# daniloceano/LorenzCycleToolkit

Measured on NVIDIA B200. Metric: LEC timesteps/s (all terms), 0.25°×37-lvl ERA5 shape; % of HBM roofline, higher is better.
Workload: dtype f32

## Files before the change

### lorenzcycletoolkit_b200/csrc/lec_engine.cu

```cuda
#include <algorithm>
#include <cmath>
#include <cstdio>
#include <cstdlib>
#include <cstring>
#include <string>
#include <vector>

#include "../../include/lec_b200.h"
#include "lec_common.cuh"
#include "lec_finalize.cuh"
#include "lec_row_moments.cuh"
#include "lec_row_tile.cuh"
#include "lec_row_narrow.cuh"
#include "lec_diag850.cuh"
#include "lec_ingest.cuh"

using namespace lec;

#ifndef LEC_TILE_DEFAULT
#define LEC_TILE_DEFAULT 1
#endif
#ifndef LEC_TILE_ROWS_DEFAULT
#define LEC_TILE_ROWS_DEFAULT 15
#endif
// ... 25 lines not shown
  int force_narrow_g = 0;
  double* d_rec = nullptr;
  double* d_fin = nullptr;
  StepDev* d_steps = nullptr;
  StepDev* h_steps = nullptr;
  cudaEvent_t ev_steps[2] = {nullptr, nullptr};
  bool steps_pending[2] = {false, false};
  int batch_parity = 0;
  int max_steps = 0, max_ny = 0;
  size_t elem = 4;
  std::vector<double> lon_deg, lat_deg, rlon, rlat, coslat, plev;
  void* stage[2][5] = {{nullptr}};
  long long stage_slots = 0;
  void* raw_stage[2] = {nullptr, nullptr};
  size_t raw_stage_bytes = 0;
  cudaStream_t s_ingest = nullptr;
  cudaEvent_t ev_raw_ready[2] = {nullptr, nullptr}, ev_raw_free[2] = {nullptr, nullptr}, ev_ingested = nullptr;
  long long raw_seq = 0;
  int* d_maps = nullptr;
  double* d_out_terms = nullptr;
  double* d_out_levels = nullptr;
  int* d_out_flags = nullptr;
  long long out_cap = 0;
  double* bnd_user = nullptr;
  double* d_out_bnd = nullptr;
  long long bnd_cap = 0;
  cudaStream_t s_copy = nullptr, s_comp = nullptr;
  cudaEvent_t ev_copied[2] = {nullptr, nullptr}, ev_done[2] = {nullptr, nullptr};
  std::vector<cudaEvent_t> ev_pool;
  int ev_used = 0;
  cudaEvent_t ev_call0 = nullptr, ev_call1 = nullptr;
  bool call_timed = false;
  bool accumulate_timing = false;
  long long launches = 0;
  lec_dispatch dispatch{};
  bool dispatched = false;
  std::string err;
};

namespace {

#if LEC_TILE_DEFAULT
const char* kVersion = "lec_b200 0.2 (sm_100a; rows=tile)";
#else
const char* kVersion = "lec_b200 0.2 (sm_100a; rows=direct)";
#endif

#define CK(call)                                                                   \
  do {                                                                             \
    cudaError_t e__ = (call);                                                      \
    if (e__ != cudaSuccess) {                                                      \
      h->err = std::string(#call) + ": " + cudaGetErrorString(e__);                \
      return LEC_ERR_CUDA;                                                         \
    }                                                                              \
  } while (0)

inline void grad_interior(const double* x, int i, double& a, double& b, double& c) {
  const double hs = x[i] - x[i - 1], hd = x[i + 1] - x[i];
  if (hs == hd) {
    a = -1.0 / (2.0 * hs); b = 0.0; c = 1.0 / (2.0 * hs);
  } else {
    a = -hd / (hs * (hd + hs)); b = (hd - hs) / (hd * hs); c = hs / (hd * (hd + hs));
  }
}

int lon_mode(const lec_handle* h) {
  const bool m64 = h->desc.dtype == LEC_F64 || h->desc.math == LEC_MATH_F64;
  const int need = m64 ? 2 : 1;
  if (h->g.lon_uniform >= need) return 0;
  return h->g.stencil_uniform >= need ? 1 : 2;
}

template <typename FT, typename CT, int VEC, bool COMP>
void launch_rows_c(const RowParams& rp, int lonw, long long grid, cudaStream_t st) {
  if (lonw == 0) lec_row_moments_kernel<FT, CT, VEC, 0, COMP><<<(unsigned)grid, kRowThreads, 0, st>>>(rp);
  else if (lonw == 1) lec_row_moments_kernel<FT, CT, VEC, 1, COMP><<<(unsigned)grid, kRowThreads, 0, st>>>(rp);
  else lec_row_moments_kernel<FT, CT, VEC, 2, COMP><<<(unsigned)grid, kRowThreads, 0, st>>>(rp);
}
template <typename FT, typename CT, int VEC>
void launch_rows_t(const RowParams& rp, int lonw, bool comp, long long grid, cudaStream_t st) {
  if constexpr (sizeof(CT) == 4) {
    if (comp) { launch_rows_c<FT, CT, VEC, true>(rp, lonw, grid, st); return; }
  }
  launch_rows_c<FT, CT, VEC, false>(rp, lonw, grid, st);
}

void launch_rows(const lec_handle* h, const RowParams& rp, bool vec, bool comp, long long grid, cudaStream_t st) {
  const bool f64 = h->desc.dtype == LEC_F64;
  const bool m64 = f64 || h->desc.math == LEC_MATH_F64;
  const int lonw = lon_mode(h);
  if (f64) {
    if (vec) launch_rows_t<double, double, 2>(rp, lonw, comp, grid, st);
    else launch_rows_t<double, double, 1>(rp, lonw, comp, grid, st);
  } else if (m64) {
    if (vec) launch_rows_t<float, double, 4>(rp, lonw, comp, grid, st);
    else launch_rows_t<float, double, 1>(rp, lonw, comp, grid, st);
  } else {
    if (vec) launch_rows_t<float, float, 4>(rp, lonw, comp, grid, st);
    else launch_rows_t<float, float, 1>(rp, lonw, comp, grid, st);
  }
}

template <typename FT, typename CT, int VEC, bool COMP, typename ST>
void launch_narrow_c(const RowParams& rp, bool table, int G, long long grid, cudaStream_t st) {
#define LEC_NARROW(LW, GG) lec_row_moments_narrow_kernel<FT, CT, VEC, LW, GG, COMP, ST><<<(unsigned)grid, kNarrowThreads, 0, st>>>(rp)
  if (table) { if (G == 16) LEC_NARROW(2, 16); else if (G == 8) LEC_NARROW(2, 8); else LEC_NARROW(2, 4); }
  else { if (G == 16) LEC_NARROW(0, 16); else if (G == 8) LEC_NARROW(0, 8); else LEC_NARROW(0, 4); }
#undef LEC_NARROW
}
template <typename FT, typename CT, int VEC, typename ST = FT>
void launch_narrow_t(const RowParams& rp, bool table, bool comp, int G, long long grid, cudaStream_t st) {
  if constexpr (sizeof(CT) == 4) {
    if (comp) { launch_narrow_c<FT, CT, VEC, true, ST>(rp, table, G, grid, st); return; }
  }
  launch_narrow_c<FT, CT, VEC, false, ST>(rp, table, G, grid, st);
}

typedef CUresult (*EncodeTiledFn)(CUtensorMap*, CUtensorMapDataType, cuuint32_t, void*, const cuuint64_t*,
                                  const cuuint64_t*, const cuuint32_t*, const cuuint32_t*, CUtensorMapInterleave,
                                  CUtensorMapSwizzle, CUtensorMapL2promotion, CUtensorMapFloatOOBfill);

EncodeTiledFn encode_tiled_fn() {
  static EncodeTiledFn fn = nullptr;
  if (!fn) {
    void* ptr = nullptr;
    cudaDriverEntryPointQueryResult qres;
    if (cudaGetDriverEntryPoint("cuTensorMapEncodeTiled", &ptr, cudaEnableDefault, &qres) == cudaSuccess &&
        qres == cudaDriverEntryPointSuccess)
      fn = reinterpret_cast<EncodeTiledFn>(ptr);
  }
  return fn;
}

bool make_map(CUtensorMap* m, const void* base, int esize, int nlon, int nlat, int nlev, int nslots, int bx, int by,
              int promo = 3) {
  EncodeTiledFn enc = encode_tiled_fn();
  if (!enc) return false;
  const cuuint64_t e = (cuuint64_t)esize;
  const cuuint64_t dims[4] = {(cuuint64_t)nlon, (cuuint64_t)nlat, (cuuint64_t)nlev, (cuuint64_t)nslots};
  const cuuint64_t strides[3] = {nlon * e, (cuuint64_t)nlat * nlon * e, (cuuint64_t)nlev * nlat * nlon * e};
  const cuuint32_t box[4] = {(cuuint32_t)bx, (cuuint32_t)by, 1, 1};
  const cuuint32_t estr[4] = {1, 1, 1, 1};
  const CUtensorMapDataType dt = esize == 8 ? CU_TENSOR_MAP_DATA_TYPE_FLOAT64
                                 : esize == 4 ? CU_TENSOR_MAP_DATA_TYPE_FLOAT32 : CU_TENSOR_MAP_DATA_TYPE_UINT16;
  return enc(m, dt, 4, const_cast<void*>(base),
             dims, strides, box, estr, CU_TENSOR_MAP_INTERLEAVE_NONE, CU_TENSOR_MAP_SWIZZLE_NONE,
             promo == 0 ? CU_TENSOR_MAP_L2_PROMOTION_NONE : promo == 1 ? CU_TENSOR_MAP_L2_PROMOTION_L2_64B
             : promo == 2 ? CU_TENSOR_MAP_L2_PROMOTION_L2_128B : CU_TENSOR_MAP_L2_PROMOTION_L2_256B,
             CU_TENSOR_MAP_FLOAT_OOB_FILL_NONE) == CUDA_SUCCESS;
}

template <typename FT, typename CT, int R, int S, bool COMP, int GL = 32, int MINB = 1, typename ST = FT>
cudaError_t launch_tile_c(const TmaMaps& maps, const RowParams& rp, int lonw, int grid, cudaStream_t st) {
  using G = TileGeom<FT, R, S, GL, ST>;
  cudaError_t e = cudaSuccess;
#define LEC_TILE_LAUNCH(LW, TB, SMEM)                                                                             \
  do {                                                                                                            \
    e = cudaFuncSetAttribute(lec_row_moments_tile_kernel<FT, CT, LW, R, S, COMP, TB, GL, MINB, ST>,          \
                             cudaFuncAttributeMaxDynamicSharedMemorySize, SMEM);                                  \
    if (e == cudaSuccess) lec_row_moments_tile_kernel<FT, CT, LW, R, S, COMP, TB, GL, MINB, ST><<<grid, G::threads, SMEM, st>>>(maps, rp); \
  } while (0)
  if constexpr (GL != 32) {
    if (lonw == 0) LEC_TILE_LAUNCH(0, false, G::smem_bytes);
    else LEC_TILE_LAUNCH(2, false, G::smem_bytes);
  } else {
    const int tab_bytes = (sizeof(ST) == sizeof(FT) ? (rp.g.nlon + 3) & ~3 : rp.pk.ntab) * 4;
    if (lonw == 0) LEC_TILE_LAUNCH(0, false, G::smem_bytes);
    else if (lonw == 1) {
      if (sizeof(CT) == 4 && sizeof(FT) == 4 && G::smem_bytes + tab_bytes <= 227 * 1024) LEC_TILE_LAUNCH(1, true, G::smem_bytes + tab_bytes);
      else LEC_TILE_LAUNCH(1, false, G::smem_bytes);
    } else LEC_TILE_LAUNCH(2, false, G::smem_bytes);
  }
#undef LEC_TILE_LAUNCH
  return e != cudaSuccess ? e : cudaGetLastError();
}

template <typename FT, typename CT>
cudaError_t launch_tile_t(const TmaMaps& maps, const RowParams& rp, int lonw, bool comp, int rows, int grid,
                          cudaStream_t st) {
  if constexpr (sizeof(CT) == 4) {
    if (comp) return launch_tile_c<FT, CT, 11, 4, true>(maps, rp, lonw, grid, st);
#ifdef LEC_TILE_ALL_SHAPES
    if (rows == 8) return launch_tile_c<FT, CT, 8, 5, false>(maps, rp, lonw, grid, st);
    if (rows == 11) return launch_tile_c<FT, CT, 11, 4, false>(maps, rp, lonw, grid, st);
    if (rows == 12) return launch_tile_c<FT, CT, 12, 4, false>(maps, rp, lonw, grid, st);
#endif
    return launch_tile_c<FT, CT, 15, 3, false>(maps, rp, lonw, grid, st);
  } else if constexpr (sizeof(FT) == 4) {
    return launch_tile_c<FT, CT, 7, 6, false>(maps, rp, lonw, grid, st);
  } else {
    return launch_tile_c<FT, CT, 11, 4, false>(maps, rp, lonw, grid, st);
  }
}

template <typename FT, typename CT>
cudaError_t launch_tile_packed(const TmaMaps& maps, const RowParams& rp, int lonw, bool comp, int grid, cudaStream_t st) {
  if constexpr (sizeof(CT) == 4) {
    if (comp) return launch_tile_c<FT, CT, 11, 7, true, 32, 1, short>(maps, rp, lonw, grid, st);
    return launch_tile_c<FT, CT, 11, 7, false, 32, 1, short>(maps, rp, lonw, grid, st);
  } else if constexpr (sizeof(FT) == 4) {
    return launch_tile_c<FT, CT, 7, 8, false, 32, 1, short>(maps, rp, lonw, grid, st);
  } else {
    return launch_tile_c<FT, CT, 11, 8, false, 32, 1, short>(maps, rp, lonw, grid, st);
  }
}

cudaEvent_t next_event(lec_handle* h) {
  if (h->ev_used == (int)h->ev_pool.size()) {
    cudaEvent_t e;
    if (cudaEventCreate(&e) != cudaSuccess) return nullptr;
    h->ev_pool.push_back(e);
  }
  return h->ev_pool[h->ev_used++];
}

int build_step(const lec_handle* h, const lec_step& s, int nslots, StepDev& d) {
  const int nlon = h->desc.nlon, nlat = h->desc.nlat;
  if (s.slot < 0 || s.slot >= nslots || s.slot_m < 0 || s.slot_m >= nslots || s.slot_p < 0 ||
      s.slot_p >= nslots)
    return LEC_ERR_BOUNDS;
  if (s.i0 < 0 || s.i1 >= nlon || s.j0 < 0 || s.j1 >= nlat) return LEC_ERR_BOUNDS;
  if (s.i1 - s.i0 < 1 || s.j1 - s.j0 < 1) return LEC_ERR_DEGENERATE;
  if (s.j1 - s.j0 + 1 > h->max_ny) return LEC_ERR_BOUNDS;
  const double* x = h->lon_deg.data();
  const double* y = h->lat_deg.data();
  const double* rl = h->rlon.data();
  const double* rp = h->rlat.data();
  d.slot = s.slot; d.slot_m = s.slot_m; d.slot_p = s.slot_p;
  d.i0 = s.i0; d.i1 = s.i1; d.j0 = s.j0; d.j1 = s.j1; d.rec_base = 0;
  const double q0 = kCp * h->g.scale[0], qv = q0 * h->g.scale[2];
  d.ct_m = q0 * s.ct_m; d.ct_p = q0 * s.ct_p; d.ct_s = q0 * (s.ct_m + s.ct_0 + s.ct_p);
  const double unit = kDeg2Rad * kRe;
  d.cxW = 1.0 / ((x[s.i0 + 1] - x[s.i0]) * unit);
  d.cxE = 1.0 / ((x[s.i1] - x[s.i1 - 1]) * unit);
  d.cyS = qv / ((y[s.j0 + 1] - y[s.j0]) * unit);
  d.cyN = qv / ((y[s.j1] - y[s.j1 - 1]) * unit);
  d.wW = 0.5 * (rl[s.i0 + 1] - rl[s.i0]);
  d.wE = 0.5 * (rl[s.i1] - rl[s.i1 - 1]);
  const double xlen = rl[s.i1] - rl[s.i0];
  const double ylen = std::sin(rp[s.j1]) - std::sin(rp[s.j0]);
  d.inv_xlen = 1.0 / xlen; d.inv_ylen = 1.0 / ylen;
  d.c1 = -1.0 / (kRe * xlen * ylen);
  d.c2 = -1.0 / (kRe * ylen);
  d.f_ct_m = (float)d.ct_m; d.f_ct_p = (float)d.ct_p; d.f_ct_s = (float)d.ct_s;
  d.f_cxW = (float)d.cxW; d.f_cxE = (float)d.cxE; d.f_cyS = (float)d.cyS; d.f_cyN = (float)d.cyN;
  d.f_wW = (float)d.wW; d.f_wE = (float)d.wE;
  d.f_wWn = h->g.wl_u != 0.0 ? (float)(d.wW / h->g.wl_u) : 0.f;
  d.f_wEn = h->g.wl_u != 0.0 ? (float)(d.wE / h->g.wl_u) : 0.f;
  d.f_pad = 0.f;
  return LEC_OK;
}

}

extern "C" {

const char* lec_version(void) { return kVersion; }

const char* lec_strerror(int code) {
  switch (code) {
    case LEC_OK: return "ok";
    case LEC_ERR_INVALID: return "invalid argument";
    case LEC_ERR_CUDA: return "CUDA runtime failure";
    case LEC_ERR_DEGENERATE: return "box axis has fewer than 2 points";
    case LEC_ERR_BOUNDS: return "box or time slot outside the prepared domain";
    case LEC_ERR_NOMEM: return "out of memory";
    default: return "unknown error";
  }
}

static thread_local std::string g_free_err;

const char* lec_last_error(lec_handle* h) { return h ? h->err.c_str() : g_free_err.c_str(); }

int64_t lec_launch_count(lec_handle* h) { return h ? h->launches : 0; }

int lec_last_dispatch(const lec_handle* h, lec_dispatch* out) {
  if (!h || !out || !h->dispatched) return LEC_ERR_INVALID;
  *out = h->dispatch;
  return LEC_OK;
}

int lec_last_transfer(lec_handle* h, int64_t out_bytes[2]) {
  if (!h || !out_bytes) return LEC_ERR_INVALID;
  out_bytes[0] = h->h2d_bytes; out_bytes[1] = h->d2h_bytes;
  return LEC_OK;
}

int lec_gradient_coefs(const double* x, int32_t n, double* a, double* b, double* c) {
  if (!x || !a || !b || !c || n < 2) return LEC_ERR_INVALID;
  bool uniform = true;
  const double h0 = x[1] - x[0];
  for (int i = 1; i + 1 < n; ++i)
    if (x[i + 1] - x[i] != h0) { uniform = false; break; }
  for (int i = 1; i + 1 < n; ++i) {
    if (uniform) { a[i] = -1.0 / (2.0 * h0); b[i] = 0.0; c[i] = 1.0 / (2.0 * h0); }
    else {
      const double hs = x[i] - x[i - 1], hd = x[i + 1] - x[i];
      a[i] = -hd / (hs * (hd + hs)); b[i] = (hd - hs) / (hd * hs); c[i] = hs / (hd * (hd + hs));
    }
  }
  a[0] = 0.0; b[0] = -1.0 / (x[1] - x[0]); c[0] = 1.0 / (x[1] - x[0]);
  a[n - 1] = -1.0 / (x[n - 1] - x[n - 2]); b[n - 1] = 1.0 / (x[n - 1] - x[n - 2]); c[n - 1] = 0.0;
  return LEC_OK;
}

int32_t lec_nearest_index(const double* coord, int32_t n, double value) {
// ... 895 lines not shown
```

### lorenzcycletoolkit_b200/csrc/lec_row_iter_tile.inc

```
    mbar_wait(fb, phase);
    if (warp_on) {
      const unsigned sbs = sb + adj;
      const unsigned a_hc = sbs + off_hc, a_t = sbs + off_t;
#if LEC_ITER_FIRST
      {
        const unsigned e0 = (unsigned)((i0 - c0 * VEC) * sizeof(ST));
        const unsigned row0 = sbs + (unsigned)(G::halo_bytes_pad + rowt * PW * sizeof(ST)) + e0;
        shT = lds_elem<ST, FT, 0>(sbs + (unsigned)(((rowt + 1) * HP + HV) * sizeof(ST)) + e0, p.pk);
        shU = lds_elem<ST, FT, 1>(row0, p.pk); shV = lds_elem<ST, FT, 2>(row0 + kTile, p.pk);
        shW = lds_elem<ST, FT, 3>(row0 + 2 * kTile, p.pk); shF = lds_elem<ST, FT, 4>(row0 + 3 * kTile, p.pk);
        cshT = CT(shT); cshU = CT(shU); cshV = CT(shV); cshW = CT(shW); cshF = CT(shF);
      }
#endif
      const int c_raw = c0 + it * GL + gl;
#if LEC_BODY_EDGE
      const bool lane_on = row_on && c_raw <= c1;
      const int col = (lane_on ? c_raw : c1) * VEC;
#else
      constexpr bool lane_on = true;
      const int col = c_raw * VEC;
#endif
      FT Tc[VEC], Tm[VEC], Tp[VEC], Tkm[VEC], Tkp[VEC], Tjm[VEC], Tjp[VEC], U[VEC], V[VEC], W[VEC], F[VEC];
      lds_row<ST, FT, VEC, 0>(a_hc, Tc, p.pk);
      FT Tl = __shfl_up_sync(0xffffffffu, Tc[VEC - 1], 1);
      FT Tr = __shfl_down_sync(0xffffffffu, Tc[0], 1);
      if (gl == 0) Tl = lds_elem<ST, FT, 0>(a_hc - (unsigned)sizeof(ST), p.pk);
      if (gl == GL - 1) Tr = lds_elem<ST, FT, 0>(a_hc + (unsigned)(VEC * sizeof(ST)), p.pk);
      lds_row<ST, FT, VEC, 0>(sbs + off_hm, Tjm, p.pk);
      lds_row<ST, FT, VEC, 0>(sbs + off_hp, Tjp, p.pk);
      lds_row<ST, FT, VEC, 0>(a_t + 4 * kTile, Tp, p.pk);
      lds_row<ST, FT, VEC, 0>(a_t + 5 * kTile, Tm, p.pk);
      lds_row<ST, FT, VEC, 0>(a_t + 6 * kTile, Tkm, p.pk);
      lds_row<ST, FT, VEC, 0>(a_t + 7 * kTile, Tkp, p.pk);
      lds_row<ST, FT, VEC, 1>(a_t, U, p.pk);
      lds_row<ST, FT, VEC, 2>(a_t + 1 * kTile, V, p.pk);
      lds_row<ST, FT, VEC, 3>(a_t + 2 * kTile, W, p.pk);
      lds_row<ST, FT, VEC, 4>(a_t + 3 * kTile, F, p.pk);
#define LEC_TAB_WL wl_tab
#define LEC_TAB_CXA p.g.cxa32
#define LEC_TAB_CXC p.g.cxc32
#define LEC_TAB_LOAD(ptr, dst) tab_load_tile<TABS && LONW == 1, VEC>(ptr, wl_s32 + (unsigned)col * 4u, dst)
#include "lec_row_body.inc"
#undef LEC_TAB_WL
#undef LEC_TAB_CXA
#undef LEC_TAB_CXC
#undef LEC_TAB_LOAD
    }
    __syncwarp();
    if (lane == 0) mbar_arrive_off<8 * NSTG>(fb);
    sb += G::stage_bytes; fb += 8;
    if (++stg == NSTG) { stg = 0; phase ^= 1; sb -= NSTG * G::stage_bytes; fb -= 8 * NSTG; }
```

### lorenzcycletoolkit_b200/csrc/lec_row_tile.cuh

```cuda
#pragma once
#include <cuda.h>

#include "lec_common.cuh"
#include "lec_packed.cuh"
#include "lec_row_moments.cuh"
#include "lec_row_narrow.cuh"

namespace lec {

struct alignas(64) TmaMaps {
  CUtensorMap t_halo;
  CUtensorMap t_plain;
  CUtensorMap u, v, w, f;
};

template <typename FT, int R, int NSTG, int GL = 32, typename ST = FT>
struct TileGeom {
  static constexpr bool I16 = sizeof(ST) != sizeof(FT);
  static constexpr int VEC = 16 / sizeof(FT);
  static constexpr int HV = I16 ? 8 : VEC;
  static constexpr int RPW = 32 / GL;
  static constexpr int ROWS = R * RPW;
  static constexpr int C = GL * VEC;
  static constexpr int PW = I16 ? C + 8 : C;
  static constexpr int HP = PW + 2 * HV;
  static_assert(HP * sizeof(ST) % 16 == 0 && PW * sizeof(ST) % 16 == 0, "TMA boxes are whole 16-byte units wide");
  static constexpr int halo_bytes = (ROWS + 2) * HP * sizeof(ST);
  static constexpr int halo_bytes_pad = (halo_bytes + 127) / 128 * 128;
  static constexpr int tile_bytes = I16 ? (ROWS * PW * (int)sizeof(ST) + 127) / 128 * 128 : ROWS * C * sizeof(ST);
  static constexpr int stage_bytes = halo_bytes_pad + 8 * tile_bytes;
  static constexpr int smem_bytes = NSTG * stage_bytes + 128;
  static constexpr int threads = (R + 1) * 32;
  static __host__ __device__ constexpr int tx_bytes(int rows) { return ((rows + 2) * HP + 8 * rows * PW) * (int)sizeof(ST); }
};

__device__ __forceinline__ unsigned smem_u32(const void* p) { return (unsigned)__cvta_generic_to_shared(p); }
__device__ __forceinline__ void mbar_init(unsigned bar, int count) {
  asm volatile("mbarrier.init.shared::cta.b64 [%0], %1;" ::"r"(bar), "r"(count) : "memory");
}
__device__ __forceinline__ void mbar_expect_tx(unsigned bar, unsigned bytes) {
  asm volatile("mbarrier.arrive.expect_tx.shared::cta.b64 _, [%0], %1;" ::"r"(bar), "r"(bytes) : "memory");
}
__device__ __forceinline__ void mbar_arrive(unsigned bar) {
  asm volatile("mbarrier.arrive.shared::cta.b64 _, [%0];" ::"r"(bar) : "memory");
}
__device__ __forceinline__ bool mbar_try_wait(unsigned bar, unsigned parity) {
  unsigned ok;
  asm volatile(
      "{\n .reg .pred p;\n mbarrier.try_wait.parity.shared::cta.b64 p, [%1], %2;\n selp.u32 %0, 1, 0, p;\n}"
      : "=r"(ok) : "r"(bar), "r"(parity) : "memory");
  return ok != 0;
}
__device__ __forceinline__ void mbar_wait(unsigned bar, unsigned parity) {
  while (!mbar_try_wait(bar, parity)) {}
}
template <int OFF>
__device__ __forceinline__ void mbar_arrive_off(unsigned bar) {
  asm volatile("mbarrier.arrive.shared::cta.b64 _, [%0+%1];" ::"r"(bar), "n"(OFF) : "memory");
}
__device__ __forceinline__ unsigned long long l2_policy_evict_first() {
  unsigned long long pol;
  asm volatile("createpolicy.fractional.L2::evict_first.b64 %0, 1.0;" : "=l"(pol));
  return pol;
}
__device__ __forceinline__ void tma_load_4d_hint(unsigned dst, const CUtensorMap* map, unsigned bar, int c0, int c1, int c2, int c3,
                                                 unsigned long long pol) {
  asm volatile(
      "cp.async.bulk.tensor.4d.shared::cluster.global.mbarrier::complete_tx::bytes.L2::cache_hint [%0], [%1, {%3, %4, %5, %6}], [%2], %7;"
      ::"r"(dst), "l"(reinterpret_cast<unsigned long long>(map)), "r"(bar), "r"(c0), "r"(c1), "r"(c2), "r"(c3), "l"(pol)
      : "memory");
}
__device__ __forceinline__ void tma_load_4d(unsigned dst, const CUtensorMap* map, unsigned bar, int c0, int c1, int c2, int c3) {
  asm volatile(
      "cp.async.bulk.tensor.4d.shared::cluster.global.mbarrier::complete_tx::bytes [%0], [%1, {%3, %4, %5, %6}], [%2];"
      ::"r"(dst), "l"(reinterpret_cast<unsigned long long>(map)), "r"(bar), "r"(c0), "r"(c1), "r"(c2), "r"(c3)
      : "memory");
}

template <typename FT, int VEC>
__device__ __forceinline__ void lds_vec(unsigned a, FT (&v)[VEC]) {
  if constexpr (sizeof(FT) == 4) {
    asm volatile("ld.shared.v4.f32 {%0, %1, %2, %3}, [%4];" : "=f"(v[0]), "=f"(v[1]), "=f"(v[2]), "=f"(v[3]) : "r"(a));
  } else {
    asm volatile("ld.shared.v2.f64 {%0, %1}, [%2];" : "=d"(v[0]), "=d"(v[1]) : "r"(a));
  }
}
__device__ __forceinline__ float lds_one(unsigned a, float) {
  float v; asm volatile("ld.shared.f32 %0, [%1];" : "=f"(v) : "r"(a)); return v;
}
__device__ __forceinline__ double lds_one(unsigned a, double) {
  double v; asm volatile("ld.shared.f64 %0, [%1];" : "=d"(v) : "r"(a)); return v;
}
template <typename ST, typename FT, int VEC, int F>
__device__ __forceinline__ void lds_row(unsigned a, FT (&v)[VEC], const PackedDev& pk) {
  if constexpr (sizeof(ST) == sizeof(FT)) {
    lds_vec<FT, VEC>(a, v);
  } else if constexpr (VEC == 4) {
    unsigned lo, hi;
    asm volatile("ld.shared.v2.u32 {%0, %1}, [%2];" : "=r"(lo), "=r"(hi) : "r"(a));
    unpack_i16_vec<FT, VEC, F, true>(lo, hi, v, pk);
  } else {
    unsigned lo;
    asm volatile("ld.shared.u32 %0, [%1];" : "=r"(lo) : "r"(a));
    unpack_i16_vec<FT, VEC, F, true>(lo, 0u, v, pk);
  }
}
template <typename ST, typename FT, int F>
__device__ __forceinline__ FT lds_elem(unsigned a, const PackedDev& pk) {
  if constexpr (sizeof(ST) == sizeof(FT)) {
    return lds_one(a, FT());
  } else {
    unsigned short r;
    asm volatile("ld.shared.u16 %0, [%1];" : "=h"(r) : "r"(a));
    return unpack_i16<FT, F, true>(short(r), pk);
  }
}

template <bool SHARED, int VEC>
__device__ __forceinline__ void tab_load(const float* ptr, float (&v)[VEC]) {
  if constexpr (SHARED && VEC == 4) {
    const float4 t = *reinterpret_cast<const float4*>(ptr); v[0] = t.x; v[1] = t.y; v[2] = t.z; v[3] = t.w;
  } else {
    VecLoad<float, VEC>::ld(ptr, v);
  }
}

template <bool SHARED, int VEC>
__device__ __forceinline__ void tab_load_tile(const float* ptr, unsigned saddr, float (&v)[VEC]) {
  if constexpr (SHARED && VEC == 4) {
    asm volatile("ld.shared.v4.f32 {%0, %1, %2, %3}, [%4];" : "=f"(v[0]), "=f"(v[1]), "=f"(v[2]), "=f"(v[3]) : "r"(saddr));
  } else {
    VecLoad<float, VEC>::ld(ptr, v);
  }
}

struct TileId { int band, s, k, jt; };
__device__ __forceinline__ TileId decode_tile(unsigned id, const RowParams& p) {
  TileId t;
  unsigned jt, k, s;
  const unsigned a = p.dv_tiles.divmod(id, jt);
  const unsigned b = p.dv_lev.divmod(a, k);
  t.band = int(p.dv_steps.divmod(b, s));
  t.jt = int(jt); t.k = int(k); t.s = int(s);
  return t;
}

template <typename FT, typename CT, int LONW, int R, int NSTG, bool COMP, bool TABS, int GL = 32, int MINB = 1, typename ST = FT>
__global__ void __launch_bounds__((R + 1) * 32, MINB)
lec_row_moments_tile_kernel(const __grid_constant__ TmaMaps maps, const RowParams p) {
  using G = TileGeom<FT, R, NSTG, GL, ST>;
  constexpr int VEC = G::VEC, C = G::C, PW = G::PW, HP = G::HP, HV = G::HV, RPW = G::RPW;
  static_assert(!G::I16 || GL == 32, "int16 fields: one warp per row");
  const int trows = (GL == 32) ? R : p.tile_rows;
  extern __shared__ __align__(1024) unsigned char smem[];
  unsigned long long* bars = reinterpret_cast<unsigned long long*>(smem + NSTG * G::stage_bytes);
  const unsigned full0 = smem_u32(bars), empty0 = smem_u32(bars + NSTG);
  const int warp = threadIdx.x >> 5, lane = threadIdx.x & 31;

  if (threadIdx.x == 0) {
    for (int i = 0; i < NSTG; ++i) { mbar_init(full0 + 8 * i, 1); mbar_init(empty0 + 8 * i, R); }
    asm volatile("fence.mbarrier_init.release.cluster;" ::: "memory");
  }
  const float* wl_tab = p.g.wl32;
  if constexpr (TABS) {
    float* wl_s = reinterpret_cast<float*>(smem + G::smem_bytes);
    int ntab = p.g.nlon;
    if constexpr (sizeof(ST) != sizeof(FT)) ntab = p.pk.ntab;
    for (int i = threadIdx.x; i < ntab; i += blockDim.x) wl_s[i] = __ldg(p.g.wl32 + i);
    wl_tab = wl_s;
  }
  __syncthreads();

  const int nlev = p.g.nlev;

  if (warp == R) {
    if (lane == 0) {
      int stg = 0;
      unsigned phase = 0;
      const unsigned long long pol_stream = l2_policy_evict_first();
      for (unsigned id = blockIdx.x; id < (unsigned)p.grid; id += gridDim.x) {
        const TileId t = decode_tile(id, p);
        const StepDev* __restrict__ st = p.steps + t.s;
        const int jr = (t.band * p.tiles_per_band + t.jt) * trows;
        if (jr > st->j1 - st->j0) continue;
        const int c0 = st->i0 / VEC, c1 = st->i1 / VEC;
        const int nch = (c1 - c0 + GL) / GL;
        const unsigned tx = (unsigned)G::tx_bytes(trows);
        const unsigned tile_b = G::I16 ? (unsigned)G::tile_bytes : (unsigned)(trows * C * (int)sizeof(ST));
        const int jt0 = st->j0 + jr;
        const int k = t.k, km = k > 0 ? k - 1 : k, kp = k < nlev - 1 ? k + 1 : k;
        const int slot = st->slot, slot_m = st->slot_m, slot_p = st->slot_p;
        int col = c0 * VEC;
        if constexpr (G::I16) col &= ~7;
        for (int ch = 0; ch < nch; ++ch, col += C) {
          mbar_wait(empty0 + 8 * stg, phase ^ 1);
          const unsigned fb = full0 + 8 * stg;
          if (p.prefetch_mode & 2) {
            mbar_arrive(fb);
            if (++stg == NSTG) { stg = 0; phase ^= 1; }
            continue;
          }
          mbar_expect_tx(fb, tx);
          const unsigned base = smem_u32(smem) + (unsigned)stg * G::stage_bytes;
          tma_load_4d(base, &maps.t_halo, fb, col - HV, jt0 - 1, k, slot);
          unsigned d = base + G::halo_bytes_pad;
          if (p.prefetch_mode & 8) {
            tma_load_4d_hint(d, &maps.u, fb, col, jt0, k, slot, pol_stream); d += tile_b;
            tma_load_4d_hint(d, &maps.v, fb, col, jt0, k, slot, pol_stream); d += tile_b;
            tma_load_4d_hint(d, &maps.w, fb, col, jt0, k, slot, pol_stream); d += tile_b;
            tma_load_4d_hint(d, &maps.f, fb, col, jt0, k, slot, pol_stream); d += tile_b;
          } else {
            tma_load_4d(d, &maps.u, fb, col, jt0, k, slot); d += tile_b;
            tma_load_4d(d, &maps.v, fb, col, jt0, k, slot); d += tile_b;
            tma_load_4d(d, &maps.w, fb, col, jt0, k, slot); d += tile_b;
            tma_load_4d(d, &maps.f, fb, col, jt0, k, slot); d += tile_b;
          }
          tma_load_4d(d, &maps.t_plain, fb, col, jt0, k, slot_p); d += tile_b;
          tma_load_4d(d, &maps.t_plain, fb, col, jt0, k, slot_m); d += tile_b;
          tma_load_4d(d, &maps.t_plain, fb, col, jt0, km, slot); d += tile_b;
          tma_load_4d(d, &maps.t_plain, fb, col, jt0, kp, slot);
          if (++stg == NSTG) { stg = 0; phase ^= 1; }
        }
      }
    }
    return;
  }

  const unsigned sbase0 = smem_u32(smem);
  const int gl = lane & (GL - 1);
  const int rowt = warp * RPW + lane / GL;
  const unsigned off_hc = (unsigned)(((rowt + 1) * HP + HV + gl * VEC) * sizeof(ST));
  const unsigned off_t = (unsigned)(G::halo_bytes_pad + (rowt * PW + gl * VEC) * sizeof(ST));
  const unsigned kTile = G::I16 ? (unsigned)G::tile_bytes : (unsigned)(trows * C * (int)sizeof(ST));
  unsigned sb = sbase0, fb = full0;
  int stg = 0;
  unsigned phase = 0;
  [[maybe_unused]] unsigned wl_s32 = 0;
  if constexpr (TABS) wl_s32 = smem_u32(smem + G::smem_bytes);
  for (unsigned id = blockIdx.x; id < (unsigned)p.grid; id += gridDim.x) {
    const TileId t = decode_tile(id, p);
    const StepDev* __restrict__ st = p.steps + t.s;
    const int i0 = st->i0, i1 = st->i1, j0 = st->j0, j1 = st->j1;
    const int jrel0 = (t.band * p.tiles_per_band + t.jt) * trows;
    if (jrel0 > j1 - j0) continue;
    const bool warp_on = (warp * RPW < trows) && (jrel0 + warp * RPW <= j1 - j0) && !(p.prefetch_mode & 4);
    const bool row_on = warp_on && (rowt < trows) && (jrel0 + rowt <= j1 - j0);
    const int jrel = row_on ? jrel0 + rowt : j1 - j0;
    const int j = j0 + jrel;
    const int k = t.k;
    const int c0 = i0 / VEC, c1 = i1 / VEC;
    const int niter = (c1 - c0 + GL) / GL;
    const unsigned adj = G::I16 ? (unsigned)(((c0 * VEC) & 7) * (int)sizeof(ST)) : 0u;

    RowSetup<CT, LONW> rs;
    rs.init(p, st, j, k, j0, j1);
    const RowCoefS<CT>& rc = rs.rc;
    const CT cxa_u = rs.cxa_u, cxc_u = rs.cxc_u, cxW = rs.cxW, cxE = rs.cxE, wW = rs.wW, wE = rs.wE;
    [[maybe_unused]] const double fxd = rs.fxd;
    const bool box_aligned = (i0 % VEC == 0) && ((i1 + 1) % VEC == 0);
    const unsigned off_hm = (j > j0) ? off_hc - (unsigned)(HP * sizeof(ST)) : off_hc;
    const unsigned off_hp = (j < j1) ? off_hc + (unsigned)(HP * sizeof(ST)) : off_hc;

    FT shT = FT(0), shU = FT(0), shV = FT(0), shW = FT(0), shF = FT(0);
    CT cshT = CT(0), cshU = CT(0), cshV = CT(0), cshW = CT(0), cshF = CT(0);
    CT S[R_NSUM], Cc[R_NLIN];
#pragma unroll
    for (int n = 0; n < R_NSUM; ++n) S[n] = CT(0);
#pragma unroll
    for (int n = 0; n < R_NLIN; ++n) Cc[n] = CT(0);
    double* __restrict__ rec = p.rec + (((long long)t.s * nlev + k) * p.max_ny + jrel) * LEC_NREC;


    {
      const int it = 0;
#define LEC_BODY_EDGE 1
#define LEC_ITER_FIRST 1
#include "lec_row_iter_tile.inc"
#undef LEC_ITER_FIRST
#undef LEC_BODY_EDGE
    }
    for (int it = 1; it < niter - 1; ++it) {
#define LEC_BODY_EDGE 0
#define LEC_ITER_FIRST 0
#include "lec_row_iter_tile.inc"
#undef LEC_ITER_FIRST
#undef LEC_BODY_EDGE
    }
    if (niter > 1) {
      const int it = niter - 1;
#define LEC_BODY_EDGE 1
#define LEC_ITER_FIRST 0
#include "lec_row_iter_tile.inc"
#undef LEC_ITER_FIRST
#undef LEC_BODY_EDGE
    }

    if (warp_on) {
      double Sd[R_NSUM];
#pragma unroll
      for (int n = 0; n < R_NSUM; ++n) Sd[n] = double(S[n]);
      if constexpr (sizeof(CT) == 4 && COMP) {
#pragma unroll
        for (int n = 0; n < R_NLIN; ++n) Sd[n] += double(Cc[n]);
      }
      if constexpr (GL == 32) {
        double tot = butterfly_reduce<R_NSUM>(Sd, lane);
        if (LONW == 0) tot *= p.g.wl_u;
        const int idx = bitrev5(lane);
        if (idx < R_NSUM) rec[idx] = tot;
      } else {
        constexpr int NOUT = (R_NSUM + GL - 1) / GL;
        double tot[NOUT];
        butterfly_reduce_seg<R_NSUM, GL>(Sd, gl, tot);
        if (row_on) {
          const int r = bitrev_group<GL>(gl);
#pragma unroll
          for (int m = 0; m < NOUT; ++m) {
            const int idx = r + m * GL;
            if (idx < R_NSUM) rec[idx] = (LONW == 0) ? tot[m] * p.g.wl_u : tot[m];
          }
        }
      }
      if (row_on && gl == 1) {
        rec[R_SH_T] = double(shT); rec[R_SH_U] = double(shU); rec[R_SH_V] = double(shV);
        rec[R_SH_W] = double(shW); rec[R_SH_F] = double(shF);
      }
    }
  }
}

}
```

Baseline: 6240.

## Precompute per-tile row setup in producer warp and release stages early

When one warp handles each row, the producer warp now decodes each tile and computes the per-row coefficient setup (RowSetup) itself. It writes these into a double-buffered shared-memory header that consumer warps read after the first stage's barrier wait, instead of each consumer recomputing the setup from global step data between tiles. Consumer warps also release a ring stage right after loading their registers, before the arithmetic, so the next TMA can be issued sooner. The mbarrier try_wait gains a suspend-time hint. This adds shared memory and extra producer-side synchronisation for header reuse, and the more intricate barrier protocol raises the risk of hangs.

```diff
diff --git a/lorenzcycletoolkit_b200/csrc/lec_engine.cu b/lorenzcycletoolkit_b200/csrc/lec_engine.cu
--- a/lorenzcycletoolkit_b200/csrc/lec_engine.cu
+++ b/lorenzcycletoolkit_b200/csrc/lec_engine.cu
@@ -201,7 +201,7 @@
 
 template <typename FT, typename CT, int R, int S, bool COMP, int GL = 32, int MINB = 1, typename ST = FT>
 cudaError_t launch_tile_c(const TmaMaps& maps, const RowParams& rp, int lonw, int grid, cudaStream_t st) {
-  using G = TileGeom<FT, R, S, GL, ST>;
+  using G = TileGeom<FT, R, S, GL, ST, CT>;
   cudaError_t e = cudaSuccess;
 #define LEC_TILE_LAUNCH(LW, TB, SMEM)                                                                             \
   do {                                                                                                            \
diff --git a/lorenzcycletoolkit_b200/csrc/lec_row_iter_tile.inc b/lorenzcycletoolkit_b200/csrc/lec_row_iter_tile.inc
--- a/lorenzcycletoolkit_b200/csrc/lec_row_iter_tile.inc
+++ b/lorenzcycletoolkit_b200/csrc/lec_row_iter_tile.inc
@@ -1,4 +1,6 @@
+#if !LEC_ITER_FIRST
     mbar_wait(fb, phase);
+#endif
     if (warp_on) {
       const unsigned sbs = sb + adj;
       const unsigned a_hc = sbs + off_hc, a_t = sbs + off_t;
@@ -36,6 +38,10 @@
       lds_row<ST, FT, VEC, 2>(a_t + 1 * kTile, V, p.pk);
       lds_row<ST, FT, VEC, 3>(a_t + 2 * kTile, W, p.pk);
       lds_row<ST, FT, VEC, 4>(a_t + 3 * kTile, F, p.pk);
+      if constexpr (EARLY_RELEASE) {
+        __syncwarp();
+        if (lane == 0) mbar_arrive_off<8 * NSTG>(fb);
+      }
 #define LEC_TAB_WL wl_tab
 #define LEC_TAB_CXA p.g.cxa32
 #define LEC_TAB_CXC p.g.cxc32
@@ -46,7 +52,9 @@
 #undef LEC_TAB_CXC
 #undef LEC_TAB_LOAD
     }
-    __syncwarp();
-    if (lane == 0) mbar_arrive_off<8 * NSTG>(fb);
+    if (!EARLY_RELEASE || !warp_on) {
+      __syncwarp();
+      if (lane == 0) mbar_arrive_off<8 * NSTG>(fb);
+    }
     sb += G::stage_bytes; fb += 8;
     if (++stg == NSTG) { stg = 0; phase ^= 1; sb -= NSTG * G::stage_bytes; fb -= 8 * NSTG; }
diff --git a/lorenzcycletoolkit_b200/csrc/lec_row_tile.cuh b/lorenzcycletoolkit_b200/csrc/lec_row_tile.cuh
--- a/lorenzcycletoolkit_b200/csrc/lec_row_tile.cuh
+++ b/lorenzcycletoolkit_b200/csrc/lec_row_tile.cuh
@@ -14,7 +14,7 @@
   CUtensorMap u, v, w, f;
 };
 
-template <typename FT, int R, int NSTG, int GL = 32, typename ST = FT>
+template <typename FT, int R, int NSTG, int GL = 32, typename ST = FT, typename CT = FT>
 struct TileGeom {
   static constexpr bool I16 = sizeof(ST) != sizeof(FT);
   static constexpr int VEC = 16 / sizeof(FT);
@@ -29,7 +29,11 @@
   static constexpr int halo_bytes_pad = (halo_bytes + 127) / 128 * 128;
   static constexpr int tile_bytes = I16 ? (ROWS * PW * (int)sizeof(ST) + 127) / 128 * 128 : ROWS * C * sizeof(ST);
   static constexpr int stage_bytes = halo_bytes_pad + 8 * tile_bytes;
-  static constexpr int smem_bytes = NSTG * stage_bytes + 128;
+  static constexpr bool HDR = GL == 32;
+  static constexpr int hdr_row_bytes = 16 * (int)sizeof(CT);
+  static constexpr int hdr_bytes = HDR ? 64 + ROWS * hdr_row_bytes : 0;
+  static constexpr int smem_bytes = NSTG * stage_bytes + 128 + 2 * hdr_bytes;
+  static_assert(smem_bytes <= 227 * 1024, "ring, barriers and headers fit the shared memory of a CTA");
   static constexpr int threads = (R + 1) * 32;
   static __host__ __device__ constexpr int tx_bytes(int rows) { return ((rows + 2) * HP + 8 * rows * PW) * (int)sizeof(ST); }
 };
@@ -44,11 +48,20 @@
 __device__ __forceinline__ void mbar_arrive(unsigned bar) {
   asm volatile("mbarrier.arrive.shared::cta.b64 _, [%0];" ::"r"(bar) : "memory");
 }
+#ifndef LEC_MBAR_SUSPEND_NS
+#define LEC_MBAR_SUSPEND_NS 10000000
+#endif
 __device__ __forceinline__ bool mbar_try_wait(unsigned bar, unsigned parity) {
   unsigned ok;
+#if LEC_MBAR_SUSPEND_NS > 0
+  asm volatile(
+      "{\n .reg .pred p;\n mbarrier.try_wait.parity.shared::cta.b64 p, [%1], %2, %3;\n selp.u32 %0, 1, 0, p;\n}"
+      : "=r"(ok) : "r"(bar), "r"(parity), "n"(LEC_MBAR_SUSPEND_NS) : "memory");
+#else
   asm volatile(
       "{\n .reg .pred p;\n mbarrier.try_wait.parity.shared::cta.b64 p, [%1], %2;\n selp.u32 %0, 1, 0, p;\n}"
       : "=r"(ok) : "r"(bar), "r"(parity) : "memory");
+#endif
   return ok != 0;
 }
 __device__ __forceinline__ void mbar_wait(unsigned bar, unsigned parity) {
@@ -134,6 +147,52 @@
   }
 }
 
+struct TileHdr {
+  int i0, i1, j0, j1;
+  int jrel0, c0, c1, niter;
+  int flags, pad;
+  long long rec0;
+  int k, slot, slot_m, slot_p;
+};
+static_assert(sizeof(TileHdr) == 64, "the header rows start at byte 64");
+constexpr int kHdrBoxAligned = 1, kHdrEnd = 2;
+
+__device__ __forceinline__ int lds_s32(unsigned a) {
+  int v; asm volatile("ld.shared.s32 %0, [%1];" : "=r"(v) : "r"(a)); return v;
+}
+__device__ __forceinline__ int4 lds_s32x4(unsigned a) {
+  int4 v;
+  asm volatile("ld.shared.v4.s32 {%0, %1, %2, %3}, [%4];" : "=r"(v.x), "=r"(v.y), "=r"(v.z), "=r"(v.w) : "r"(a));
+  return v;
+}
+__device__ __forceinline__ long long lds_s64(unsigned a) {
+  long long v; asm volatile("ld.shared.s64 %0, [%1];" : "=l"(v) : "r"(a)); return v;
+}
+
+template <typename CT, int LONW>
+__device__ __forceinline__ void hdr_put_row(unsigned char* row, const RowSetup<CT, LONW>& rs) {
+  CT* v = reinterpret_cast<CT*>(row);
+  v[0] = rs.rc.ct_m; v[1] = rs.rc.ct_p; v[2] = rs.rc.ct_s; v[3] = rs.rc.cy_m; v[4] = rs.rc.cy_p;
+  v[5] = rs.rc.s_m; v[6] = rs.rc.s_p; v[7] = rs.rc.s_s; v[8] = rs.rc.fx;
+  v[9] = rs.cxa_u; v[10] = rs.cxc_u; v[11] = rs.cxW; v[12] = rs.cxE; v[13] = rs.wW; v[14] = rs.wE; v[15] = CT(0);
+}
+template <typename CT, int LONW>
+__device__ __forceinline__ void hdr_get_row(unsigned a, RowSetup<CT, LONW>& rs) {
+  constexpr int NV = 16 / sizeof(CT);
+  CT v[16];
+#pragma unroll
+  for (int n = 0; n < 16 / NV; ++n) {
+    CT t[NV];
+    lds_vec<CT, NV>(a + 16 * n, t);
+#pragma unroll
+    for (int e = 0; e < NV; ++e) v[n * NV + e] = t[e];
+  }
+  rs.rc.ct_m = v[0]; rs.rc.ct_p = v[1]; rs.rc.ct_s = v[2]; rs.rc.cy_m = v[3]; rs.rc.cy_p = v[4];
+  rs.rc.s_m = v[5]; rs.rc.s_p = v[6]; rs.rc.s_s = v[7]; rs.rc.fx = v[8];
+  rs.cxa_u = v[9]; rs.cxc_u = v[10]; rs.cxW = v[11]; rs.cxE = v[12]; rs.wW = v[13]; rs.wE = v[14];
+  rs.fxd = sizeof(CT) == 8 ? double(v[8]) : 0.0;
+}
+
 struct TileId { int band, s, k, jt; };
 __device__ __forceinline__ TileId decode_tile(unsigned id, const RowParams& p) {
   TileId t;
@@ -148,7 +207,7 @@
 template <typename FT, typename CT, int LONW, int R, int NSTG, bool COMP, bool TABS, int GL = 32, int MINB = 1, typename ST = FT>
 __global__ void __launch_bounds__((R + 1) * 32, MINB)
 lec_row_moments_tile_kernel(const __grid_constant__ TmaMaps maps, const RowParams p) {
-  using G = TileGeom<FT, R, NSTG, GL, ST>;
+  using G = TileGeom<FT, R, NSTG, GL, ST, CT>;
   constexpr int VEC = G::VEC, C = G::C, PW = G::PW, HP = G::HP, HV = G::HV, RPW = G::RPW;
   static_assert(!G::I16 || GL == 32, "int16 fields: one warp per row");
   const int trows = (GL == 32) ? R : p.tile_rows;
@@ -172,12 +231,104 @@
   __syncthreads();
 
   const int nlev = p.g.nlev;
+  const unsigned hdr0 = full0 + 128;
 
   if (warp == R) {
-    if (lane == 0) {
+    const unsigned long long pol_stream = l2_policy_evict_first();
+    const unsigned tx = (unsigned)G::tx_bytes(trows);
+    const unsigned tile_b = G::I16 ? (unsigned)G::tile_bytes : (unsigned)(trows * C * (int)sizeof(ST));
+    auto issue = [&](int stg, unsigned fb, int col, int jt0, int k, int slot, int slot_m, int slot_p) {
+      if (p.prefetch_mode & 2) {
+        mbar_arrive(fb);
+        return;
+      }
+      const int km = k > 0 ? k - 1 : k, kp = k < nlev - 1 ? k + 1 : k;
+      mbar_expect_tx(fb, tx);
+      const unsigned base = smem_u32(smem) + (unsigned)stg * G::stage_bytes;
+      tma_load_4d(base, &maps.t_halo, fb, col - HV, jt0 - 1, k, slot);
+      unsigned d = base + G::halo_bytes_pad;
+      if (p.prefetch_mode & 8) {
+        tma_load_4d_hint(d, &maps.u, fb, col, jt0, k, slot, pol_stream); d += tile_b;
+        tma_load_4d_hint(d, &maps.v, fb, col, jt0, k, slot, pol_stream); d += tile_b;
+        tma_load_4d_hint(d, &maps.w, fb, col, jt0, k, slot, pol_stream); d += tile_b;
+        tma_load_4d_hint(d, &maps.f, fb, col, jt0, k, slot, pol_stream); d += tile_b;
+      } else {
+        tma_load_4d(d, &maps.u, fb, col, jt0, k, slot); d += tile_b;
+        tma_load_4d(d, &maps.v, fb, col, jt0, k, slot); d += tile_b;
+        tma_load_4d(d, &maps.w, fb, col, jt0, k, slot); d += tile_b;
+        tma_load_4d(d, &maps.f, fb, col, jt0, k, slot); d += tile_b;
+      }
+      tma_load_4d(d, &maps.t_plain, fb, col, jt0, k, slot_p); d += tile_b;
+      tma_load_4d(d, &maps.t_plain, fb, col, jt0, k, slot_m); d += tile_b;
+      tma_load_4d(d, &maps.t_plain, fb, col, jt0, km, slot); d += tile_b;
+      tma_load_4d(d, &maps.t_plain, fb, col, jt0, kp, slot);
+    };
+    if constexpr (G::HDR) {
+      unsigned q = 0, q1 = 0, q2 = 0, nhdr = 0;
+      unsigned id = blockIdx.x;
+      TileId t{};
+      const StepDev* __restrict__ st = p.steps;
+      int jrel0 = 0;
+      bool end = false;
+      RowSetup<CT, LONW> rs;
+      auto build_next = [&]() {
+        for (; id < (unsigned)p.grid; id += gridDim.x) {
+          t = decode_tile(id, p);
+          st = p.steps + t.s;
+          jrel0 = (t.band * p.tiles_per_band + t.jt) * R;
+          if (jrel0 <= st->j1 - st->j0) break;
+        }
+        end = id >= (unsigned)p.grid;
+        if (!end && lane >= 1 && lane <= R) {
+          const int j0 = st->j0, j1 = st->j1;
+          const int jrel = (jrel0 + lane - 1 <= j1 - j0) ? jrel0 + lane - 1 : j1 - j0;
+          rs.init(p, st, j0 + jrel, t.k, j0, j1);
+        }
+      };
+      if (lane != 0) build_next();
+      for (;;) {
+        const int stg = (int)(q % NSTG);
+        const unsigned fb = full0 + 8 * stg, par = (q / NSTG) & 1;
+        if (lane == 0) {
+          mbar_wait(empty0 + 8 * stg, par ^ 1);
+          if (nhdr >= 2 && q2 + NSTG > q) mbar_wait(empty0 + 8 * (q2 % NSTG), (q2 / NSTG) & 1);
+        }
+        __syncwarp();
+        TileHdr* h = reinterpret_cast<TileHdr*>(smem + NSTG * G::stage_bytes + 128 + (nhdr & 1) * G::hdr_bytes);
+        if (lane == 1) {
+          const int i0 = st->i0, i1 = st->i1;
+          h->flags = end ? kHdrEnd : ((i0 % VEC == 0) && ((i1 + 1) % VEC == 0)) ? kHdrBoxAligned : 0;
+          h->i0 = i0; h->i1 = i1; h->j0 = st->j0; h->j1 = st->j1;
+          h->jrel0 = jrel0; h->c0 = i0 / VEC; h->c1 = i1 / VEC; h->niter = (i1 / VEC - i0 / VEC + GL) / GL;
+          h->rec0 = ((long long)t.s * nlev + t.k) * p.max_ny * LEC_NREC;
+          h->k = t.k; h->slot = st->slot; h->slot_m = st->slot_m; h->slot_p = st->slot_p;
+        }
+        if (!end && lane >= 1 && lane <= R) hdr_put_row(reinterpret_cast<unsigned char*>(h) + 64 + (lane - 1) * G::hdr_row_bytes, rs);
+        __syncwarp();
+        if (h->flags & kHdrEnd) {
+          if (lane == 0) mbar_arrive(fb);
+          break;
+        }
+        const int nch = h->niter;
+        if (lane == 0) {
+          const int k = h->k, slot = h->slot, slot_m = h->slot_m, slot_p = h->slot_p, jt0 = h->j0 + h->jrel0;
+          int col = h->c0 * VEC;
+          if constexpr (G::I16) col &= ~7;
+          for (int ch = 0; ch < nch; ++ch, col += C) {
+            const unsigned qc = q + ch;
+            const int sc = (int)(qc % NSTG);
+            if (ch > 0) mbar_wait(empty0 + 8 * sc, ((qc / NSTG) & 1) ^ 1);
+            issue(sc, full0 + 8 * sc, col, jt0, k, slot, slot_m, slot_p);
+          }
+        } else {
+          id += gridDim.x;
+          build_next();
+        }
+        q2 = q1; q1 = q; q += nch; ++nhdr;
+      }
+    } else if (lane == 0) {
       int stg = 0;
       unsigned phase = 0;
-      const unsigned long long pol_stream = l2_policy_evict_first();
       for (unsigned id = blockIdx.x; id < (unsigned)p.grid; id += gridDim.x) {
         const TileId t = decode_tile(id, p);
         const StepDev* __restrict__ st = p.steps + t.s;
@@ -185,40 +336,11 @@
         if (jr > st->j1 - st->j0) continue;
         const int c0 = st->i0 / VEC, c1 = st->i1 / VEC;
         const int nch = (c1 - c0 + GL) / GL;
-        const unsigned tx = (unsigned)G::tx_bytes(trows);
-        const unsigned tile_b = G::I16 ? (unsigned)G::tile_bytes : (unsigned)(trows * C * (int)sizeof(ST));
-        const int jt0 = st->j0 + jr;
-        const int k = t.k, km = k > 0 ? k - 1 : k, kp = k < nlev - 1 ? k + 1 : k;
-        const int slot = st->slot, slot_m = st->slot_m, slot_p = st->slot_p;
+        const int jt0 = st->j0 + jr, slot = st->slot, slot_m = st->slot_m, slot_p = st->slot_p;
         int col = c0 * VEC;
-        if constexpr (G::I16) col &= ~7;
         for (int ch = 0; ch < nch; ++ch, col += C) {
           mbar_wait(empty0 + 8 * stg, phase ^ 1);
-          const unsigned fb = full0 + 8 * stg;
-          if (p.prefetch_mode & 2) {
-            mbar_arrive(fb);
-            if (++stg == NSTG) { stg = 0; phase ^= 1; }
-            continue;
-          }
-          mbar_expect_tx(fb, tx);
-          const unsigned base = smem_u32(smem) + (unsigned)stg * G::stage_bytes;
-          tma_load_4d(base, &maps.t_halo, fb, col - HV, jt0 - 1, k, slot);
-          unsigned d = base + G::halo_bytes_pad;
-          if (p.prefetch_mode & 8) {
-            tma_load_4d_hint(d, &maps.u, fb, col, jt0, k, slot, pol_stream); d += tile_b;
-            tma_load_4d_hint(d, &maps.v, fb, col, jt0, k, slot, pol_stream); d += tile_b;
-            tma_load_4d_hint(d, &maps.w, fb, col, jt0, k, slot, pol_stream); d += tile_b;
-            tma_load_4d_hint(d, &maps.f, fb, col, jt0, k, slot, pol_stream); d += tile_b;
-          } else {
-            tma_load_4d(d, &maps.u, fb, col, jt0, k, slot); d += tile_b;
-            tma_load_4d(d, &maps.v, fb, col, jt0, k, slot); d += tile_b;
-            tma_load_4d(d, &maps.w, fb, col, jt0, k, slot); d += tile_b;
-            tma_load_4d(d, &maps.f, fb, col, jt0, k, slot); d += tile_b;
-          }
-          tma_load_4d(d, &maps.t_plain, fb, col, jt0, k, slot_p); d += tile_b;
-          tma_load_4d(d, &maps.t_plain, fb, col, jt0, k, slot_m); d += tile_b;
-          tma_load_4d(d, &maps.t_plain, fb, col, jt0, km, slot); d += tile_b;
-          tma_load_4d(d, &maps.t_plain, fb, col, jt0, kp, slot);
+          issue(stg, full0 + 8 * stg, col, jt0, t.k, slot, slot_m, slot_p);
           if (++stg == NSTG) { stg = 0; phase ^= 1; }
         }
       }
@@ -232,32 +354,57 @@
   const unsigned off_hc = (unsigned)(((rowt + 1) * HP + HV + gl * VEC) * sizeof(ST));
   const unsigned off_t = (unsigned)(G::halo_bytes_pad + (rowt * PW + gl * VEC) * sizeof(ST));
   const unsigned kTile = G::I16 ? (unsigned)G::tile_bytes : (unsigned)(trows * C * (int)sizeof(ST));
+  constexpr bool EARLY_RELEASE = GL == 32 && !G::I16;
   unsigned sb = sbase0, fb = full0;
   int stg = 0;
   unsigned phase = 0;
   [[maybe_unused]] unsigned wl_s32 = 0;
   if constexpr (TABS) wl_s32 = smem_u32(smem + G::smem_bytes);
-  for (unsigned id = blockIdx.x; id < (unsigned)p.grid; id += gridDim.x) {
-    const TileId t = decode_tile(id, p);
-    const StepDev* __restrict__ st = p.steps + t.s;
-    const int i0 = st->i0, i1 = st->i1, j0 = st->j0, j1 = st->j1;
-    const int jrel0 = (t.band * p.tiles_per_band + t.jt) * trows;
-    if (jrel0 > j1 - j0) continue;
+  [[maybe_unused]] unsigned id = blockIdx.x, hs = 0;
+  for (;;) {
+    int i0, i1, j0, j1, jrel0, c0, c1, niter;
+    bool box_aligned;
+    long long rec0;
+    [[maybe_unused]] const StepDev* __restrict__ st = p.steps;
+    [[maybe_unused]] int k = 0;
+    [[maybe_unused]] unsigned ha = 0;
+    if constexpr (G::HDR) {
+      mbar_wait(fb, phase);
+      ha = hdr0 + hs * (unsigned)G::hdr_bytes;
+      hs ^= 1;
+      const int flags = lds_s32(ha + 32);
+      if (flags & kHdrEnd) break;
+      const int4 ha0 = lds_s32x4(ha), ha1 = lds_s32x4(ha + 16);
+      i0 = ha0.x; i1 = ha0.y; j0 = ha0.z; j1 = ha0.w;
+      jrel0 = ha1.x; c0 = ha1.y; c1 = ha1.z; niter = ha1.w;
+      box_aligned = (flags & kHdrBoxAligned) != 0;
+      rec0 = lds_s64(ha + 40);
+    } else {
+      if (id >= (unsigned)p.grid) break;
+      const TileId t = decode_tile(id, p);
+      id += gridDim.x;
+      st = p.steps + t.s;
+      k = t.k;
+      i0 = st->i0; i1 = st->i1; j0 = st->j0; j1 = st->j1;
+      jrel0 = (t.band * p.tiles_per_band + t.jt) * trows;
+      if (jrel0 > j1 - j0) continue;
+      c0 = i0 / VEC; c1 = i1 / VEC;
+      niter = (c1 - c0 + GL) / GL;
+      box_aligned = (i0 % VEC == 0) && ((i1 + 1) % VEC == 0);
+      rec0 = ((long long)t.s * nlev + k) * p.max_ny * LEC_NREC;
+    }
     const bool warp_on = (warp * RPW < trows) && (jrel0 + warp * RPW <= j1 - j0) && !(p.prefetch_mode & 4);
     const bool row_on = warp_on && (rowt < trows) && (jrel0 + rowt <= j1 - j0);
     const int jrel = row_on ? jrel0 + rowt : j1 - j0;
     const int j = j0 + jrel;
-    const int k = t.k;
-    const int c0 = i0 / VEC, c1 = i1 / VEC;
-    const int niter = (c1 - c0 + GL) / GL;
     const unsigned adj = G::I16 ? (unsigned)(((c0 * VEC) & 7) * (int)sizeof(ST)) : 0u;
 
     RowSetup<CT, LONW> rs;
-    rs.init(p, st, j, k, j0, j1);
+    if constexpr (G::HDR) hdr_get_row(ha + 64 + (unsigned)(rowt * G::hdr_row_bytes), rs);
+    else rs.init(p, st, j, k, j0, j1);
     const RowCoefS<CT>& rc = rs.rc;
     const CT cxa_u = rs.cxa_u, cxc_u = rs.cxc_u, cxW = rs.cxW, cxE = rs.cxE, wW = rs.wW, wE = rs.wE;
     [[maybe_unused]] const double fxd = rs.fxd;
-    const bool box_aligned = (i0 % VEC == 0) && ((i1 + 1) % VEC == 0);
     const unsigned off_hm = (j > j0) ? off_hc - (unsigned)(HP * sizeof(ST)) : off_hc;
     const unsigned off_hp = (j < j1) ? off_hc + (unsigned)(HP * sizeof(ST)) : off_hc;
 
@@ -268,7 +415,8 @@
     for (int n = 0; n < R_NSUM; ++n) S[n] = CT(0);
 #pragma unroll
     for (int n = 0; n < R_NLIN; ++n) Cc[n] = CT(0);
-    double* __restrict__ rec = p.rec + (((long long)t.s * nlev + k) * p.max_ny + jrel) * LEC_NREC;
+    double* __restrict__ rec = p.rec + rec0 + (long long)jrel * LEC_NREC;
+    if constexpr (!G::HDR) mbar_wait(fb, phase);
 
 
     {
```

New measurement: 6085, median of 6. 0.975x the previous value.
